# chronoxor/CppServer

Measured on AMD Instinct MI355X. Metric: WS payload mask/unmask GiB/s (device-resident), batched 64KiB frames, higher is better.
Workload: dtype u8; 1 GPU; C2 unmask-only: 4096 masked binary frames x 65536 B payload, one key per frame; parallelism=independent batch per GPU (dp1), frames=4096, payload_bytes_per_frame=65536, wire_bytes=268492800

## Files before the change

### cppserver_amd/csrc/wsg_kernels.hip

```cpp
#include "wsg_device.h"

namespace wsg {

namespace {

typedef uint64_t v4u64 __attribute__((ext_vector_type(4)));

constexpr int MAXF = 4;

#ifndef WSG_ENC_NT_SRC
#define WSG_ENC_NT_SRC 0
#endif
#ifndef WSG_ENC_NT_HI
#define WSG_ENC_NT_HI 1
#endif
#ifndef WSG_DIAG_ENC
#define WSG_DIAG_ENC 0
#endif
#ifndef WSG_DIAG
#define WSG_DIAG 0
#endif
#ifndef WSG_DIAG_FAN
#define WSG_DIAG_FAN 0
#endif
#ifndef WSG_DIAG_NOINFO
#define WSG_DIAG_NOINFO 0
#endif
#ifndef WSG_DEC_WAVES
#define WSG_DEC_WAVES 1
#endif
#ifndef WSG_DEC_RELOAD
#define WSG_DEC_RELOAD 1
#endif
#ifndef WSG_FAN_PERIOD
#define WSG_FAN_PERIOD 1
#endif
#ifndef WSG_FAN_UNROLL
#define WSG_FAN_UNROLL 1
#endif
#ifndef WSG_FAN_CAP
#define WSG_FAN_CAP 0
#endif
#ifndef WSG_FAN_MANY_WPC
#define WSG_FAN_MANY_WPC 46
#endif
#ifndef WSG_FAN_MANY_WPB
#define WSG_FAN_MANY_WPB 0
#endif
#ifndef WSG_FAN_KV
#define WSG_FAN_KV 2
#endif

__device__ __forceinline__ v4u ld16_sys(const void* p)
{
    v4u r;
    asm volatile("global_load_dwordx4 %0, %1, off sc0 sc1\n\ts_waitcnt vmcnt(0)" : "=v"(r) : "v"(p) : "memory");
    return r;
}

#ifndef WSG_OUT_SC1
#define WSG_OUT_SC1 0
#endif
#ifndef WSG_OUT_AUX
#define WSG_OUT_AUX 16
#endif
#ifndef WSG_ENC_SC1
#define WSG_ENC_SC1 0
#endif
#ifndef WSG_FAN_SC1
#define WSG_FAN_SC1 1
#endif
struct OutTile {
    uint8_t* p;
    bool sc1;
    __amdgpu_buffer_rsrc_t rs;
    __device__ __forceinline__ OutTile(uint8_t* base, uint32_t bytes, bool write_through = WSG_OUT_SC1 != 0)
        : p(base), sc1(write_through)
    {
        if (sc1)
            rs = __builtin_amdgcn_make_buffer_rsrc(base, 0, bytes, 0x00020000);
    }
    __device__ __forceinline__ void put(uint32_t o, v4u v) const
    {
        if (sc1)
            __builtin_amdgcn_raw_buffer_store_b128(v, rs, o, 0, WSG_OUT_AUX);
        else
            st16nt(p + o, v);
    }
};

#ifndef WSG_STAGE_FPL
#define WSG_STAGE_FPL 2
#endif
constexpr int SPL = WSG_STAGE_FPL;
constexpr int LDSF = BLOCK * SPL;

__device__ __forceinline__ void fill_tiles_wave(uint32_t* tile_first, uint64_t lo, uint64_t hi, uint32_t frame)
{
    const uint32_t lane = threadIdx.x & 63;
    constexpr uint64_t kShort = 16;
    if (hi > lo && hi - lo <= kShort)
        for (uint64_t t = lo; t < hi; ++t)
            tile_first[t] = frame;
    uint64_t pending = __ballot(hi > lo + kShort);
    while (pending) {
        const int j = __builtin_ctzll(pending);
        pending &= pending - 1;
        const uint64_t a = lane_bcast(lo, j), b = lane_bcast(hi, j);
        const uint32_t fj = __builtin_amdgcn_readlane(frame, j);
        for (uint64_t t = a + lane; t < b; t += 64)
            tile_first[t] = fj;
    }
}

__device__ __forceinline__ uint64_t lane_off(int u) { return (uint64_t(u) * BLOCK + threadIdx.x) * CHUNK; }

}


namespace {

__device__ __forceinline__ uint64_t fs_at(const uint64_t* __restrict__ fs, uint32_t n, int64_t i)
{
    return fs[min<int64_t>(i, int64_t(n) - 1)];
}

__device__ __forceinline__ int64_t search8(const uint64_t* __restrict__ fs, uint32_t a, uint32_t b, uint64_t p)
{
    while (a < b) {
        const uint32_t step = (b - a + 8) / 9;
        uint64_t v[8];
#pragma unroll
        for (int k = 0; k < 8; ++k)
            v[k] = fs[min(a - 1 + step * (k + 1), b - 1)];
        uint32_t na = a, nb = b;
#pragma unroll
        for (int k = 0; k < 8; ++k) {
            const uint32_t ix = min(a - 1 + step * (k + 1), b - 1);
            if (ix >= na && ix < nb) {
                if (v[k] <= p)
                    na = ix + 1;
                else
                    nb = ix;
            }
        }
        a = na;
        b = nb;
    }
    return int64_t(a) - 1;
}

struct TileLoc {
    int64_t f0;
    uint32_t first;
    uint64_t st[MAXF + 1];
};

__device__ __forceinline__ uint64_t tile_guess(uint32_t n, double frames_per_byte, uint64_t base)
{
    return uni(min(uint64_t(double(base) * frames_per_byte), uint64_t(n - 1)));
}

__device__ __forceinline__ uint32_t probe_index(uint64_t g, uint32_t stride, uint32_t n, int k)
{
    const int64_t i = int64_t(g) + int64_t(k - 32) * int64_t(stride);
    return uint32_t(max<int64_t>(0, min<int64_t>(i, int64_t(n) - 1)));
}

__device__ __forceinline__ void locate(const uint64_t* __restrict__ fs, uint32_t n, uint64_t g, uint32_t stride,
                                       uint64_t probe, uint64_t base, TileLoc& L)
{
    uint64_t w[MAXF + 2];
#pragma unroll
    for (int k = 0; k < MAXF + 2; ++k) {
        const uint64_t x = fs_at(fs, n, int64_t(g) + k);
        w[k] = (g + k < n) ? x : ~uint64_t(0);
    }
    if (w[0] <= base && base < w[1]) {
        L.f0 = int64_t(g);
        L.first = uint32_t(g);
#pragma unroll
        for (int k = 0; k <= MAXF; ++k)
            L.st[k] = w[k];
        return;
    }
    const uint64_t below = __ballot(probe <= base);
    const int m = __builtin_popcountll(below);
    uint32_t a = m > 0 ? probe_index(g, stride, n, m - 1) + 1 : 0;
    uint32_t b = m < 64 ? probe_index(g, stride, n, m) : n;
    if (m == 0 && probe_index(g, stride, n, 0) == 0)
        b = 0;
    L.f0 = search8(fs, a, b, base);
    L.first = uint32_t(L.f0 < 0 ? 0 : L.f0);
#pragma unroll
    for (int k = 0; k <= MAXF; ++k) {
        const uint64_t x = fs_at(fs, n, int64_t(L.first) + k);
        L.st[k] = (uint64_t(L.first) + k < n) ? x : ~uint64_t(0);
    }
}

struct Seg {
    uint32_t lo, hi, kr;
};

__device__ __forceinline__ Seg tile_seg(uint64_t po, uint64_t pe, uint32_t key, uint64_t base, uint32_t span)
{
    Seg s;
    s.lo = po <= base ? 0u : uint32_t(min<uint64_t>(po - base, span));
    s.hi = pe <= base ? 0u : uint32_t(min<uint64_t>(pe - base, span));
    if (s.hi < s.lo)
        s.hi = s.lo;
    s.kr = key_rot(key, uint32_t(base - po));
    return s;
}

__device__ __forceinline__ v4u seg_xor(uint32_t o, const Seg& s)
{
    if (s.hi <= o || s.lo >= o + CHUNK)
        return v4u{0, 0, 0, 0};
    const int a = s.lo > o ? int(s.lo - o) : 0;
    const int b = s.hi < o + CHUNK ? int(s.hi - o) : int(CHUNK);
    v4u m;
#pragma unroll
    for (int d = 0; d < 4; ++d)
        m[d] = s.kr & low_bytes(b - 4 * d) & ~low_bytes(a - 4 * d);
    return m;
}

struct TileIn {
    uint64_t base, g, probe;
    v4u v[UNROLL];
};

__device__ __forceinline__ void load_tile(TileIn& T, const uint8_t* __restrict__ wire, uint64_t wire_len,
                                          const uint64_t* __restrict__ fs, uint32_t n, double frames_per_byte,
                                          uint32_t stride, uint64_t base)
{
    T.base = base;
    T.g = tile_guess(n, frames_per_byte, base);
#if WSG_DIAG == 7
    T.probe = 0;
#else
    T.probe = fs[probe_index(T.g, stride, n, int(threadIdx.x & 63))];
#endif
    __builtin_amdgcn_sched_barrier(0);
    const uint64_t last_blk = (wire_len - 1) & ~uint64_t(CHUNK - 1);
#pragma unroll
    for (int u = 0; u < UNROLL; ++u)
        T.v[u] = ld16nt(wire + min(base + lane_off(u), last_blk));
}

__device__ __forceinline__ void process_tile(const TileIn& T, const uint8_t* __restrict__ wire, uint8_t* out,
                                             uint64_t wire_len, const uint64_t* __restrict__ fs, uint32_t n,
                                             uint32_t stride)
{
    const uint64_t base = T.base;
    const uint64_t tend = min(base + TILE, wire_len);
    const uint32_t span = uint32_t(tend - base);
    const bool full = span == TILE;
    const uint64_t g = T.g;
    const uint64_t probe = T.probe;
    const v4u* v = T.v;
    auto keep_probe = [&]() {
        if (n == 0 && probe == ~uint64_t(0))
            out[0] = 0;
    };
    TileLoc L;
    locate(fs, n, g, stride, probe, base, L);
    int c = 0;
#pragma unroll
    for (int k = 0; k <= MAXF; ++k) {
        const bool touches = uint64_t(L.first) + k < n && (k == 0 ? L.f0 >= 0 || L.st[0] < tend : L.st[k] < tend);
        if (touches && c == k)
            c = k + 1;
    }

    if (WSG_DIAG == 5 || (full && c <= MAXF)) {
        Seg S[MAXF];
#pragma unroll
        for (int k = 0; k < MAXF; ++k) {
            S[k] = Seg{0, 0, 0};
            if (k < c) {
                wsg_recv_info r;
                const uint64_t lim = (uint64_t(L.first) + k + 1 < n) ? L.st[k + 1] : wire_len;
                frame_parse(wire, wire_len, L.st[k], lim, r);
                const Seg g = tile_seg(r.payload_off, r.payload_off + r.len, r.key, base, span);
                S[k] = Seg{uni(g.lo), uni(g.hi), uni(g.kr)};
            }
        }
#if WSG_DIAG == 5
        if (true) {
#else
        if (S[0].lo == 0 && S[0].hi == TILE) {
#endif
            const OutTile ot(out + base, uint32_t(TILE));
#pragma unroll
            for (int u = 0; u < UNROLL; ++u)
                ot.put(uint32_t(lane_off(u)), v[u] ^ S[0].kr);
            keep_probe();
            return;
        }
        const OutTile ot(out + base, uint32_t(TILE));
#pragma unroll
        for (int u = 0; u < UNROLL; ++u) {
            const uint32_t o = uint32_t(lane_off(u));
            uint32_t kx = 0;
            bool cut = false;
#pragma unroll
            for (int k = 0; k < MAXF; ++k) {
                kx = (S[k].lo <= o && o + CHUNK <= S[k].hi) ? S[k].kr : kx;
                cut |= (S[k].lo > o && S[k].lo < o + CHUNK) || (S[k].hi > o && S[k].hi < o + CHUNK);
            }
            v4u x = v4u{kx, kx, kx, kx};
            if (cut) {
                x = seg_xor(o, S[0]);
#pragma unroll
                for (int k = 1; k < MAXF; ++k)
                    x |= seg_xor(o, S[k]);
            }
            ot.put(o, v[u] ^ x);
        }
        keep_probe();
        return;
    }

    __shared__ uint32_t s_lo[LDSF], s_hi[LDSF], s_kr[LDSF];
    __shared__ uint32_t s_wcnt[BLOCK / 64];
    auto stage = [&](uint64_t r0, int& cnt, bool& more) {
        uint64_t sj[SPL], lim[SPL];
        bool touch[SPL];
#pragma unroll
        for (int q = 0; q < SPL; ++q) {
            const uint64_t fi = r0 + uint64_t(q) * BLOCK + threadIdx.x;
            sj[q] = ~uint64_t(0);
            lim[q] = wire_len;
            if (fi < n) {
                sj[q] = fs[fi];
                lim[q] = fi + 1 < n ? fs[fi + 1] : wire_len;
            }
            touch[q] = fi < n && (fi == L.first || sj[q] < tend);
        }
        uint32_t wc = 0;
#pragma unroll
        for (int q = 0; q < SPL; ++q)
            wc += uint32_t(__builtin_popcountll(__ballot(touch[q])));
        const bool last_more = __ballot(threadIdx.x == BLOCK - 1 && touch[SPL - 1] &&
                                        r0 + uint64_t(LDSF) < n && lim[SPL - 1] < tend) != 0;
        __syncthreads();
        if ((threadIdx.x & 63) == 0)
            s_wcnt[threadIdx.x >> 6] = wc | (last_more ? 0x80000000u : 0u);
        __syncthreads();
        cnt = 0;
        more = false;
#pragma unroll
        for (int w = 0; w < BLOCK / 64; ++w) {
            const uint32_t x = s_wcnt[w];
            cnt += int(x & 0x7FFFFFFFu);
            more = more || (x >> 31) != 0;
        }
#pragma unroll 1
        for (int q = 0; q < SPL; ++q) {
            const int slot = q * BLOCK + int(threadIdx.x);
            if (slot < cnt) {
                wsg_recv_info r;
                frame_parse(wire, wire_len, sj[q], lim[q], r);
                const Seg g = tile_seg(r.payload_off, r.payload_off + r.len, r.key, base, span);
                s_lo[slot] = g.lo;
                s_hi[slot] = g.hi;
                s_kr[slot] = g.kr;
            }
        }
        __syncthreads();
    };
    auto chunk_xor = [&](uint32_t o, int cnt) {
        int lo = 0, hi = cnt;
#pragma unroll 1
        while (lo < hi) {
            const int mid = (lo + hi) >> 1;
            if (s_hi[mid] <= o)
                lo = mid + 1;
            else
                hi = mid;
        }
        v4u x = {0, 0, 0, 0};
#pragma unroll 1
        for (int j = lo; j < cnt && s_lo[j] < o + CHUNK; ++j)
            x |= seg_xor(o, Seg{s_lo[j], s_hi[j], s_kr[j]});
        return x;
    };
    __shared__ v4u s_acc[UNROLL][BLOCK];
#pragma unroll 1
    for (uint64_t r0 = L.first;; r0 += LDSF) {
        int cnt;
        bool more;
        stage(r0, cnt, more);
#pragma unroll 1
        for (int u = 0; u < UNROLL; ++u) {
            const v4u x = chunk_xor(uint32_t(lane_off(u)), cnt);
            s_acc[u][threadIdx.x] = (r0 == L.first) ? x : (s_acc[u][threadIdx.x] | x);
        }
        if (!more)
            break;
    }
    {
        const OutTile ot(out + base, uint32_t(TILE));
#pragma unroll 1
        for (int u = 0; u < UNROLL; ++u) {
            const uint32_t o = uint32_t(lane_off(u));
            if (o + CHUNK <= span) {
                ot.put(o, ld16(wire + base + o) ^ s_acc[u][threadIdx.x]);
            } else if (o < span) {
                uint8_t* b = reinterpret_cast<uint8_t*>(&s_acc[u][threadIdx.x]);
#pragma unroll 1
                for (uint32_t k = 0; k < span - o; ++k)
                    out[base + o + k] = uint8_t(wire[base + o + k] ^ b[k]);
            }
        }
    }
    keep_probe();
}

}

__global__ __launch_bounds__(BLOCK) __attribute__((amdgpu_waves_per_eu(WSG_DEC_WAVES))) void k_decode(const uint8_t* __restrict__ wire, uint8_t* out, uint64_t wire_len,
                                                  const uint64_t* __restrict__ fs, uint32_t n, double frames_per_byte,
                                                  uint32_t stride, wsg_recv_info* __restrict__ info,
                                                  unsigned long long* err, uint64_t num_tiles)
{
    {
        const uint64_t fstride = uint64_t(gridDim.x) * BLOCK;
        for (uint64_t i0 = uint64_t(blockIdx.x) * BLOCK + (threadIdx.x & ~63u); i0 < n && !WSG_DIAG_NOINFO;
             i0 += fstride) {
            const uint64_t i = i0 + (threadIdx.x & 63u);
            if (i < n) {
                wsg_recv_info r;
                const int e = frame_parse(wire, wire_len, fs[i], i + 1 < n ? fs[i + 1] : wire_len, r);
                if (e != 0)
                    latch(err, i, e);
                store_info(info + i, r);
            }
        }
    }

#if WSG_DIAG == 6
    for (uint64_t t = blockIdx.x; t < num_tiles; t += gridDim.x) {
        const uint64_t base = t * TILE;
        if (base + TILE > wire_len)
            break;
        v4u v[UNROLL];
#pragma unroll
        for (int u = 0; u < UNROLL; ++u) {
            v[u] = ld16nt(wire + base + lane_off(u));
#ifdef WSG_DIAG_ORD
            __builtin_amdgcn_sched_barrier(0);
#endif
        }
#pragma unroll
        for (int u = 0; u < UNROLL; ++u)
            st16nt(out + base + lane_off(u), v[u] ^ 0x9u);
    }
    return;
#endif
    for (uint64_t t = blockIdx.x; t < num_tiles; t += gridDim.x) {
        TileIn a;
        load_tile(a, wire, wire_len, fs, n, frames_per_byte, stride, t * TILE);
        process_tile(a, wire, out, wire_len, fs, n, stride);
    }
}


namespace {

struct Desc {
    uint64_t src_off, len;
    uint32_t key;
    int32_t status;
    uint8_t opcode;
    bool mask;
};

__device__ __forceinline__ Desc load_desc(const wsg_send_desc* d)
{
    const uint32_t* w = reinterpret_cast<const uint32_t*>(d);
    Desc r;
    r.src_off = uint64_t(w[0]) | (uint64_t(w[1]) << 32);
    r.len = uint64_t(w[2]) | (uint64_t(w[3]) << 32);
    r.key = w[4];
    r.status = int32_t(w[5]);
    r.opcode = uint8_t(w[6]);
    r.mask = ((w[6] >> 8) & 0xFFu) != 0;
    return r;
}
static_assert(offsetof(wsg_send_desc, key) == 16 && offsetof(wsg_send_desc, opcode) == 24 &&
                  offsetof(wsg_send_desc, mask) == 25,
              "wsg_send_desc layout");

struct StagedBlocks {
    const v4u* s;
    const uint8_t* base;
    __device__ v4u operator()(const uint8_t* p) const { return s[(p - base) >> 4]; }
};

__device__ __forceinline__ v4u shr_bytes(v4u x, uint64_t o)
{
    return o >= CHUNK ? v4u{0, 0, 0, 0} : funnel(x, v4u{0, 0, 0, 0}, uint32_t(o));
}
__device__ __forceinline__ v4u shl_bytes(v4u x, uint64_t s)
{
    return s == 0 ? x : s >= CHUNK ? v4u{0, 0, 0, 0} : funnel(v4u{0, 0, 0, 0}, x, uint32_t(CHUNK - s));
}
__device__ __forceinline__ v4u low_bytes(uint64_t n)
{
    const uint64_t lo = n >= 8 ? ~uint64_t(0) : (uint64_t(1) << (8 * n)) - 1;
    const uint64_t hi = n >= 16 ? ~uint64_t(0) : n <= 8 ? 0 : (uint64_t(1) << (8 * (n - 8))) - 1;
    return v4u{uint32_t(lo), uint32_t(lo >> 32), uint32_t(hi), uint32_t(hi >> 32)};
}

__device__ __forceinline__ void edge_chunk2(const FrameRec& R, v4u head, uint64_t p, uint8_t* __restrict__ wire)
{
    if (p + CHUNK <= R.off)
        return;
    v4u w = p >= R.off ? shr_bytes(head, p - R.off) : shl_bytes(head, R.off - p);
    const int64_t data_len = int64_t(R.end - R.data_w);
    const int64_t rel = int64_t(p) - int64_t(R.data_w);
    if (rel < data_len && rel + int64_t(CHUNK) > 0) {
        const v4u d = fan_window(R.src, uint64_t(data_len), rel);
        const uint32_t kw = key_rot(R.key, uint32_t(p - R.pw));
        const uint64_t lo = p < R.data_w ? R.data_w - p : 0;
        const uint64_t hi = R.end - p < CHUNK ? R.end - p : CHUNK;
        w |= (d ^ v4u{kw, kw, kw, kw}) & (low_bytes(hi) & ~low_bytes(lo));
    }
    const uint32_t o_lo = p < R.off ? uint32_t(R.off - p) : 0u;
    const uint32_t o_hi = R.end - p < CHUNK ? uint32_t(R.end - p) : uint32_t(CHUNK);
    if ((o_lo == 0 && o_hi == CHUNK) || (WSG_DIAG_ENC & 4)) {
        st16nt(wire + p, w);
        return;
    }
    uint32_t* w32 = reinterpret_cast<uint32_t*>(wire + p);
#pragma unroll
    for (uint32_t k = 0; k < 4; ++k) {
        const uint32_t b0 = 4 * k, b1 = b0 + 4;
        if (b0 >= o_lo && b1 <= o_hi) {
            w32[k] = w[k];
        } else {
            for (uint32_t j = max(b0, o_lo); j < min(b1, o_hi); ++j)
                wire[p + j] = uint8_t(w[k] >> (8 * (j - b0)));
        }
    }
}

template <bool NT>
struct Piece {
    FrameRec R;
    uint64_t lo = 0, hi = 0;
    uint32_t s = 0;
    uint32_t kw = 0;
    bool live = false;
    uint32_t dmask = 0;
    v4u a[EU], b[EU];

    __device__ __forceinline__ void load(const FrameRec& rec, uint64_t k, bool exists)
    {
        R = rec;
        const uint32_t lane = threadIdx.x & 63;
        lo = (R.off & ~(PIECE_ALIGN - 1)) + k * PIECE;
        live = exists && lo < R.end;
        hi = min(lo + PIECE, R.end);
        s = (WSG_DIAG_ENC & 2) ? 0u
                                : uint32_t((reinterpret_cast<uintptr_t>(R.src) + (lo - R.data_w)) & 15u);
        kw = key_rot(R.key, uint32_t(lo - R.pw));
#pragma unroll
        for (int u = 0; u < EU; ++u) {
            const uint64_t p = lo + (uint64_t(u) * 64 + lane) * CHUNK;
            const bool d = live && p < hi && p >= R.data_w && p + CHUNK <= R.end;
            dmask |= uint32_t(d) << u;
            const uint8_t* a0 = R.src + (int64_t(p - R.data_w) - int64_t(s));
            a[u] = d ? (NT ? ld16nt(a0) : ld16(a0)) : v4u{0, 0, 0, 0};
        }
#pragma unroll
        for (int u = 0; u < EU; ++u) {
            const uint64_t p = lo + (uint64_t(u) * 64 + lane) * CHUNK;
            const uint8_t* a0 = R.src + (int64_t(p - R.data_w) - int64_t(s));
            b[u] = ((dmask >> u) & 1u) && s ? ((NT && WSG_ENC_NT_HI) ? ld16nt(a0 + CHUNK) : ld16(a0 + CHUNK))
                                          : v4u{0, 0, 0, 0};
        }
    }

    __device__ __forceinline__ void store(uint8_t* __restrict__ wire) const
    {
        if (!live)
            return;
        const uint32_t lane = threadIdx.x & 63;
        const OutTile ot(wire + lo, uint32_t(PIECE), WSG_ENC_SC1 != 0);
        v4u head = {0, 0, 0, 0};
        if (lo < R.data_w)
            head = frame_head(R);
#pragma unroll
        for (int u = 0; u < EU; ++u) {
            const uint64_t p = lo + (uint64_t(u) * 64 + lane) * CHUNK;
            if ((dmask >> u) & 1u) {
                ot.put(uint32_t(p - lo), (s ? funnel(a[u], b[u], s) : a[u]) ^ kw);
            } else if (p < hi && !(WSG_DIAG_ENC & 1)) {
                edge_chunk2(R, head, p, wire);
            }
        }
    }
};

__device__ __forceinline__ uint64_t pieces_of(uint64_t frame_bytes)
{
    return (frame_bytes + PIECE_ALIGN - 1 + PIECE - 1) / PIECE;
}

}

template <bool PIECES>
__global__ __launch_bounds__(BLOCK) void k_encode_scan_local(const wsg_send_desc* __restrict__ desc, uint32_t n,
                                                             uint64_t* __restrict__ wire_off,
                                                             uint32_t* __restrict__ piece_start,
                                                             uint64_t* __restrict__ block_sums,
                                                             uint64_t* __restrict__ block_psums)
{
    const uint64_t first = uint64_t(blockIdx.x) * SCAN_ITEMS;
    uint64_t sz[SCAN_PER_LANE];
#pragma unroll
    for (int k = 0; k < SCAN_PER_LANE; ++k) {
        const uint64_t i = first + uint64_t(k) * BLOCK + threadIdx.x;
        sz[k] = 0;
        if (i < n) {
            const Desc d = load_desc(desc + i);
            const SendGeom g = send_geom(d.opcode, d.mask, d.len, d.status);
            sz[k] = g.hdr + g.body;
        }
    }
    uint64_t run = 0, run_p = 0;
#pragma unroll
    for (int k = 0; k < SCAN_PER_LANE; ++k) {
        const uint64_t i = first + uint64_t(k) * BLOCK + threadIdx.x;
        uint64_t tot, tot_p = 0;
        const uint64_t ex = block_scan_ex(sz[k], OpAdd{}, &tot);
        uint64_t ex_p = 0;
        if (PIECES)
            ex_p = block_scan_ex(sz[k] ? pieces_of(sz[k]) : 0, OpAdd{}, &tot_p);
        if (i < n) {
            wire_off[i] = run + ex;
            if (PIECES)
                piece_start[i] = uint32_t(run_p + ex_p);
        }
        run += tot;
        run_p += tot_p;
    }
    if (threadIdx.x == 0) {
        block_sums[blockIdx.x] = run;
        if (PIECES)
            block_psums[blockIdx.x] = run_p;
    }
}

__global__ __launch_bounds__(BLOCK) void k_encode_scan_blocks(const uint64_t* __restrict__ block_sums,
                                                              const uint64_t* __restrict__ block_psums, uint32_t nb,
                                                              uint64_t* __restrict__ block_prefix,
                                                              uint64_t* __restrict__ block_pprefix,
                                                              uint64_t* __restrict__ wire_off,
                                                              uint32_t* __restrict__ piece_start, uint32_t n)
{
    const uint64_t carry = scan_partials(block_sums, block_prefix, nb, OpAdd{});
    const uint64_t carry_p = scan_partials(block_psums, block_pprefix, nb, OpAdd{});
    if (threadIdx.x == 0) {
        wire_off[n] = carry;
        piece_start[n] = uint32_t(carry_p);
    }
}

__global__ __launch_bounds__(BLOCK) void k_encode_finalize(const wsg_send_desc* __restrict__ desc, uint32_t n,
                                                           uint64_t* __restrict__ wire_off,
                                                           uint32_t* __restrict__ piece_start,
                                                           const uint64_t* __restrict__ block_prefix,
                                                           const uint64_t* __restrict__ block_pprefix,
                                                           uint32_t* __restrict__ piece_frame, uint64_t pieces_cap,
                                                           uint64_t wire_cap, unsigned long long* err)
{
    if (blockIdx.x * BLOCK + (threadIdx.x & ~63u) >= n)
        return;
    const uint32_t i = blockIdx.x * BLOCK + threadIdx.x;
    uint64_t lo = 0, hi = 0;
    if (i < n) {
        const wsg_send_desc d = desc[i];
        const SendGeom g = send_geom(d.opcode, d.mask != 0, d.len, d.status);
        const uint64_t off = wire_off[i] + block_prefix[i / SCAN_ITEMS];
        const uint64_t ps = piece_start[i] + block_pprefix[i / SCAN_ITEMS];
        const uint64_t end = off + g.hdr + g.body;
        wire_off[i] = off;
        piece_start[i] = uint32_t(ps);
        if (end > wire_cap)
            latch(err, i, WSG_ENOMEM);
        piece_range(ps, ps + pieces_of(g.hdr + g.body), pieces_cap, lo, hi);
    }
    fill_tiles_wave(piece_frame, lo, hi, i);
}

__global__ __launch_bounds__(BLOCK) void k_encode_mask(const uint8_t* __restrict__ payload,
                                                       const wsg_send_desc* __restrict__ desc, uint32_t n,
                                                       const uint64_t* __restrict__ wire_off,
                                                       const uint32_t* __restrict__ piece_start,
                                                       const uint32_t* __restrict__ piece_frame,
                                                       uint8_t* __restrict__ wire, uint64_t wire_cap,
                                                       uint32_t q_begin, uint32_t q_end)
{
    const uint32_t waves = gridDim.x * (BLOCK / 64);
    uint32_t q = q_begin + blockIdx.x * (BLOCK / 64) + wave_id();
    if (wire_off[n] > wire_cap)
        return;
    const uint32_t pieces = min(piece_start[n], q_end);
    struct Meta {
        Desc d;
        uint64_t off;
        uint32_t ps;
    };
    auto meta = [&](uint32_t i) { return Meta{load_desc(desc + i), wire_off[i], piece_start[i]}; };
    if (q >= pieces)
// ... 1001 lines not shown
```

Baseline: 2953 GiB/s.

## Cache tile in LDS for header parsing and interpolate segment search start

Result: no change. 2970 GiB/s (median of 2 runs) (+0.6%).

```diff
diff --git a/cppserver_amd/csrc/wsg_kernels.hip b/cppserver_amd/csrc/wsg_kernels.hip
--- a/cppserver_amd/csrc/wsg_kernels.hip
+++ b/cppserver_amd/csrc/wsg_kernels.hip
@@ -29,8 +29,8 @@
 #ifndef WSG_DEC_WAVES
 #define WSG_DEC_WAVES 1
 #endif
-#ifndef WSG_DEC_RELOAD
-#define WSG_DEC_RELOAD 1
+#ifndef WSG_DEC_INTERP
+#define WSG_DEC_INTERP 1
 #endif
 #ifndef WSG_FAN_PERIOD
 #define WSG_FAN_PERIOD 1
@@ -326,6 +326,21 @@
 
     __shared__ uint32_t s_lo[LDSF], s_hi[LDSF], s_kr[LDSF];
     __shared__ uint32_t s_wcnt[BLOCK / 64];
+    __shared__ v4u s_tile[UNROLL][BLOCK];
+#pragma unroll
+    for (int u = 0; u < UNROLL; ++u) {
+        const uint32_t o = uint32_t(lane_off(u));
+        v4u d = v[u];
+        if (!full)
+            d = o < span ? ld16(wire + base + o) : v4u{0, 0, 0, 0};
+        s_tile[u][threadIdx.x] = d;
+    }
+    auto tile_block = [&](uint64_t a) {
+        const uint64_t d = a - base;
+        if (d < TILE)
+            return (&s_tile[0][0])[d >> 4];
+        return ld16(wire + a);
+    };
     auto stage = [&](uint64_t r0, int& cnt, bool& more) {
         uint64_t sj[SPL], lim[SPL];
         bool touch[SPL];
@@ -358,12 +373,12 @@
             cnt += int(x & 0x7FFFFFFFu);
             more = more || (x >> 31) != 0;
         }
-#pragma unroll 1
+#pragma unroll
         for (int q = 0; q < SPL; ++q) {
             const int slot = q * BLOCK + int(threadIdx.x);
             if (slot < cnt) {
                 wsg_recv_info r;
-                frame_parse(wire, wire_len, sj[q], lim[q], r);
+                frame_parse_b(tile_block, wire_len, sj[q], lim[q], r);
                 const Seg g = tile_seg(r.payload_off, r.payload_off + r.len, r.key, base, span);
                 s_lo[slot] = g.lo;
                 s_hi[slot] = g.hi;
@@ -374,6 +389,17 @@
     };
     auto chunk_xor = [&](uint32_t o, int cnt) {
         int lo = 0, hi = cnt;
+#if WSG_DEC_INTERP
+        {
+            const int j = int(o * uint32_t(cnt) / uint32_t(TILE));
+            const int a = max(j - 2, 0), b = min(j + 2, cnt);
+            const uint32_t ea = s_hi[max(a - 1, 0)], eb = s_hi[min(b, LDSF - 1)];
+            if (a > 0 && ea <= o)
+                lo = a;
+            if (b < cnt && eb > o)
+                hi = b;
+        }
+#endif
 #pragma unroll 1
         while (lo < hi) {
             const int mid = (lo + hi) >> 1;
@@ -388,7 +414,7 @@
             x |= seg_xor(o, Seg{s_lo[j], s_hi[j], s_kr[j]});
         return x;
     };
-    __shared__ v4u s_acc[UNROLL][BLOCK];
+    const OutTile ot(out + base, uint32_t(TILE));
 #pragma unroll 1
     for (uint64_t r0 = L.first;; r0 += LDSF) {
         int cnt;
@@ -396,26 +422,22 @@
         stage(r0, cnt, more);
 #pragma unroll 1
         for (int u = 0; u < UNROLL; ++u) {
-            const v4u x = chunk_xor(uint32_t(lane_off(u)), cnt);
-            s_acc[u][threadIdx.x] = (r0 == L.first) ? x : (s_acc[u][threadIdx.x] | x);
+            const uint32_t o = uint32_t(lane_off(u));
+            const v4u d = s_tile[u][threadIdx.x] ^ chunk_xor(o, cnt);
+            if (more) {
+                s_tile[u][threadIdx.x] = d;
+            } else if (o + CHUNK <= span) {
+                ot.put(o, d);
+            } else if (o < span) {
+                s_tile[u][threadIdx.x] = d;
+                const uint8_t* b = reinterpret_cast<const uint8_t*>(&s_tile[u][threadIdx.x]);
+#pragma unroll 1
+                for (uint32_t k = 0; k < span - o; ++k)
+                    out[base + o + k] = b[k];
+            }
         }
         if (!more)
             break;
-    }
-    {
-        const OutTile ot(out + base, uint32_t(TILE));
-#pragma unroll 1
-        for (int u = 0; u < UNROLL; ++u) {
-            const uint32_t o = uint32_t(lane_off(u));
-            if (o + CHUNK <= span) {
-                ot.put(o, ld16(wire + base + o) ^ s_acc[u][threadIdx.x]);
-            } else if (o < span) {
-                uint8_t* b = reinterpret_cast<uint8_t*>(&s_acc[u][threadIdx.x]);
-#pragma unroll 1
-                for (uint32_t k = 0; k < span - o; ++k)
-                    out[base + o + k] = uint8_t(wire[base + o + k] ^ b[k]);
-            }
-        }
     }
     keep_probe();
 }
```
